# skywoodsz/qm_control

Measured on NVIDIA H100. Metric: mpc_wbc_iters_per_s, higher is better.
Workload: dtype f64

## Files before the change

### qm_control_b200/csrc/kernels/mpc_kernels.cu

```cuda
#include <cstdlib>
#include "mpc_api.cuh"
#include "mpc_device.cuh"
#include "node_eval.cuh"
#include "wlinalg.cuh"

namespace qmb {

#ifndef QMB_LQ_WARPS
#define QMB_LQ_WARPS 4
#endif
#ifndef QMB_LQ_MINB
#define QMB_LQ_MINB 4
#endif
constexpr int LQ_WARPS = QMB_LQ_WARPS, LS_WARPS = 4, SETUP_WARPS = 4;
enum { MST_ITER_CAP = 1, MST_OVERFLOW = 2, MST_NAN = 4, MST_NOT_PD = 8, MST_NO_STEP = 16, MST_CONVERGED = 32, MST_NEG_DT = 64 };

__device__ __forceinline__ double interval_start(double t, int ev) { return ev == 2 ? t + WEAK_EPS : t; }
__device__ __forceinline__ double interval_end(double t, int ev) { return ev == 1 ? t - WEAK_EPS : t; }
__device__ __forceinline__ int clamp_events(int ne) { return ne < 0 ? 0 : (ne > EMAX ? EMAX : ne); }
__device__ __forceinline__ int clamp_targets(int nk) { return nk < 1 ? 1 : (nk > KMAX ? KMAX : nk); }
__device__ __forceinline__ int flag_mask(int mode) { int m = 0; for (int i = 0; i < 4; ++i) if (contact_flag(mode, i)) m |= 1 << i; return m; }

struct SetupIdx { int iu, ix; double au, ax; };
__host__ __device__ inline size_t setup_smem_per_warp(int nmax) { return (size_t)nmax * (8 + 8 + 4 + sizeof(SetupIdx) + 4) + 8 * EMAX + 64; }
// ... 259 lines not shown
  const double dyn_ss = warp_sum(bb * bb);
  if (lane < NX) {
    const int c = lane; double a1[9], out[9];
#pragma unroll
    for (int q = 0; q < 9; ++q) a1[q] = sm.A1r[q * NX + c];
#pragma unroll
    for (int r = 0; r < 9; ++r) { const double* a2 = sm.Ar + r * NX; double aa = 0.0;
#pragma unroll
      for (int q = 0; q < 9; ++q) aa = fma(a2[3 + q], a1[q], aa);
      out[r] = dt * (w1 * a1[r] + w2 * (a2[c] + cdt * aa));
      if (c < 12) { double b1 = 0.0, b2 = 0.0; if (r < 3) { b1 = b1v[r < 3 ? r : 0]; b2 = b2v[r < 3 ? r : 0]; } double ab = a2[c % 3] * imass;
#pragma unroll
        for (int q = 0; q < 3; ++q) ab += a2[3 + q] * b1v[q]; lt.BrdF[r * 12 + c] = dt * (w1 * b1 + w2 * (b2 + cdt * ab)); }
      else if (r < 3) lt.BrdJ[r * NJ + c - 12] = dt * w2 * cdt * a2[c]; }
#pragma unroll
    for (int r = 0; r < 9; ++r) sm.A1r[r * NX + c] = out[r];
  }
  __syncwarp();
  double* tl = sg + ST_TAIL; int32_t* si = reinterpret_cast<int32_t*>(tl + T_INT);
  if (lane < NX) {
    const int r = lane; double bt = lt.bvec[r];
    if (r >= 3 && r < 6) {
      double* arow = sm.A1r + (r - 3) * NX; double acc[12];
#pragma unroll
      for (int i = 0; i < 4; ++i) { const LegWs& L = sm.leg[i];
#pragma unroll
        for (int c = 0; c < 12; ++c) acc[c] = 0.0;
        for (int j = 0; j < 3; ++j) if (L.dep[j]) { const double coef = lt.BrdJ[(r - 3) * NJ + L.first + j]; bt += coef * L.Pe[j];
#pragma unroll
          for (int c = 0; c < 12; ++c) acc[c] = fma(coef, L.Px[j][c], acc[c]); }
#pragma unroll
        for (int c = 0; c < 12; ++c) arow[sup_col(c, L.first)] += acc[c];
      }
    }
    if (r >= 12 && r < 24) {
      const int i = foot_of_leg_joint(lfp, r - 12); const LegWs& L = sm.leg[i]; const int j = (r - 12) % 3;
      if (L.dep[j]) bt += dtw * L.Pe[j];
    }
    if (r < 3) for (int f = 0; f < 4; ++f) bt += (dtw * imass) * sm.Pe_full[3 * f + r];
    if (r >= 3 && r < 12) for (int f = 0; f < 4; ++f) if (!sm.leg[f].stance) for (int a = 0; a < 3; ++a) bt += lt.BrdF[(r - 3) * 12 + 3 * f + a] * sm.Pe_full[3 * f + a];
    tl[T_b + r] = bt;
    if (r >= 3 && r < 12) sg[ST_AR + (r - 3) * LDX + NX] = bt;
  }
  if (lane >= 3 && lane < 12) sm.A1r[(lane - 3) * NX + lane] += 1.0;
  __syncwarp();
#pragma unroll
  for (int r = 0; r < 9; ++r) { if (lane < NX) sg[ST_AR + r * LDX + lane] = sm.A1r[r * NX + lane]; else if (lane == 31) sg[ST_AR + r * LDX + 31] = 0.0; }
  for (int e = lane; e < 36; e += 32) sg[ST_AR + (e >> 2) * LDX + 32 + (e & 3)] = 0.0;
  for (int e = lane; e < 144; e += 32) { const int j12 = e / 12, c = e - 12 * j12; const LegWs& L = sm.leg[foot_of_leg_joint(lfp, j12)]; const int j = j12 % 3; tl[T_PXJ + e] = L.dep[j] ? L.Px[j][c] : 0.0; }
  for (int e = lane; e < 9 * LDB; e += 32) {
    const int rr = e / LDB, a = e - rr * LDB; const int r = 3 + rr; double v = 0.0;
    if (a < m) { const int fa = sm.free_idx[a];
      if (fa < 12) v = lt.BrdF[rr * 12 + fa];
      else if (r < 6) { v = lt.BrdJ[rr * NJ + fa - 12];
        if (fa < 24) { const LegWs& L = sm.leg[foot_of_leg_joint(lfp, fa - 12)]; if (!L.stance) { const int jf = (fa - 12) % 3; v += lt.BrdJ[rr * NJ + L.first + L.pivot] * L.Pu2[jf > L.pivot ? jf - 1 : jf]; } } }
    }
    sg[ST_BR + e] = v;
  }
  if (lane < NX) {
    const int r = lane; double acc[NX];
    if (mdl->q_is_diag) { const double qrr = mdl->Qdiag[r];
#pragma unroll
      for (int c = 0; c < NX; ++c) acc[c] = (c == r) ? qrr : 0.0; }
    else {
#pragma unroll
      for (int c = 0; c < NX; ++c) acc[c] = mdl->Q[r * NX + c]; }
    double qv = sm.quad.qf[r];
    const int ea = ee_pos(r);
    if (ea >= 0) {
#pragma unroll
      for (int c = 0; c < 6; ++c) { acc[6 + c] += sm.quad.E[ea * 12 + c]; acc[24 + c] += sm.quad.E[ea * 12 + 6 + c]; }
    }
#pragma unroll
    for (int i = 0; i < 4; ++i) {
      const LegWs& L = sm.leg[i]; const int first = L.first;
      const int pr = (r < 6) ? r : ((r >= 9 && r < 12) ? r - 3 : ((r >= 12 + first && r < 15 + first) ? 9 + r - 12 - first : -1));
      if (pr >= 0) {
        double blk[12];
#pragma unroll
        for (int c = 0; c < 12; ++c) blk[c] = 0.0;
        double w3[3] = {0.0, 0.0, 0.0};
        for (int j = 0; j < 3; ++j) if (L.dep[j]) { const double pj = L.Px[j][pr]; qv = fma(pj, L.rs[j], qv);
#pragma unroll
          for (int a = 0; a < 3; ++a) w3[a] = fma(pj, L.Rl[3 * j + a], w3[a]); }
        for (int a = 0; a < 3; ++a) if (L.dep[a]) { const double wa = w3[a];
#pragma unroll
          for (int c = 0; c < 12; ++c) blk[c] = fma(wa, L.Px[a][c], blk[c]); }
#pragma unroll
        for (int c = 0; c < 6; ++c) acc[c] += blk[c];
#pragma unroll
        for (int c = 0; c < 3; ++c) acc[9 + c] += blk[6 + c];
#pragma unroll
        for (int l = 0; l < 4; ++l) if (first == 3 * l) {
#pragma unroll
          for (int c = 0; c < 3; ++c) acc[12 + 3 * l + c] += blk[9 + c]; }
      }
    }
    const double dq = sm.quad.qdiag[r];
#pragma unroll
    for (int c = 0; c < NX; ++c) if (r <= c) sg[ST_Q + q_row_offset(c) + r] = dt * (acc[c] + ((c == r) ? dq : 0.0));
    if (!(r & 1)) sg[ST_Q + q_row_offset(r) + r + 1] = 0.0;
    tl[T_q + r] = dt * qv;
  }
  for (int e = lane; e < 8 * 12; e += 32) tl[T_SJ + e] = 0.0;
  __syncwarp();
  if (lane < MU) {
    const int a = lane; double rt[3] = {0.0, 0.0, 0.0}; double rtil = 0.0;
    if (a < m) {
      const int fa = sm.free_idx[a]; double rv = sm.rs[fa]; int li = -1, jf = -1;
      if (fa >= 12 && fa < 24) { li = foot_of_leg_joint(lfp, fa - 12); jf = (fa - 12) % 3; }
      const bool swing_joint = li >= 0 && !sm.leg[li].stance;
      if (swing_joint) {
        const LegWs& L = sm.leg[li]; const int pv = L.pivot; const int jfi = jf > pv ? jf - 1 : jf; const double pu = L.Pu2[jfi];
        rv += pu * L.rs[pv];
        const double coef = L.Rl[3 * jf + pv]; double* Srow = tl + T_SJ + (2 * li + jfi) * 12;
        const double cf = dt * (coef + pu * L.Rl[3 * pv + pv]);
        for (int c = 0; c < 12; ++c) Srow[c] = cf * L.Px[pv][c];
      }
      rtil = dt * rv;
      if (fa >= 24) rt[0] = dt * quad_R(mdl, &sm.quad, fa, fa);
      else { const int bi = fa / 3;
        for (int jc = 0; jc < 3; ++jc) { const int fc = 3 * bi + jc; if (sm.col_of_input[fc] < 0) continue;
          double v = quad_R(mdl, &sm.quad, fa, fc);
          if (swing_joint) { const LegWs& L = sm.leg[li]; const int pv = L.pivot; const double pa = L.Pu2[jf > pv ? jf - 1 : jf], pc = L.Pu2[jc > pv ? jc - 1 : jc];
            v += pa * L.Rl[3 * pv + jc] + L.Rl[3 * jf + pv] * pc + pa * L.Rl[3 * pv + pv] * pc; }
          rt[jc] = dt * v; } }
    }
    tl[T_r + a] = rtil; tl[T_RT + 3 * a] = rt[0]; tl[T_RT + 3 * a + 1] = rt[1]; tl[T_RT + 3 * a + 2] = rt[2];
  }
  if (lane < 4) { const LegWs& L = sm.leg[lane]; tl[T_PU2 + 2 * lane] = L.Pu2[0]; tl[T_PU2 + 2 * lane + 1] = L.Pu2[1]; si[SI_PIV + lane] = L.stance ? -1 : L.pivot;
    int nf = 0; for (int jj = 0; jj < 3; ++jj) if (!L.stance && jj != L.pivot) si[SI_PCOL + 2 * lane + nf++] = L.free_col[jj]; if (L.stance) { si[SI_PCOL + 2 * lane] = -1; si[SI_PCOL + 2 * lane + 1] = -1; } }
  if (lane < MAXDEP) { const int d = lane; double pe = 0.0; int di = -1; if (d < ndep) { di = sm.dep_idx[d]; pe = sm.Pe_full[di]; } tl[T_PED + d] = pe; si[SI_DEP + d] = di; }
  if (lane < MU) si[SI_FREE + lane] = (lane < m) ? sm.free_idx[lane] : -1;
  if (lane == 0) { si[SI_TYPE] = 0; si[SI_M] = m; si[SI_NDEP] = ndep; tl[T_MISC] = dtw; tl[T_MISC + 1] = dt * cost_val; tl[T_MISC + 2] = dt * dyn_ss; tl[T_MISC + 3] = dt * eq_ss; }
}

#ifndef QMB_TMA
#define QMB_TMA 1
#endif
constexpr int RIC_THREADS = 128, RIC_NTYPE = 512;
struct RicSmem {
  double P[NX * LDX];
  double A[NX * LDX];
  double W[NX * LDX];
  double Bm[NX * LDB], PB[NX * LDB];
  double G[MU * LDG];
  double H[MU * LDH];
  double Lt[MU * MU];
  alignas(16) double tail[TAIL_DBL];
  double dx[32], dut[32], tmp[32];
  double red[RIC_THREADS / 32][4];
  alignas(8) unsigned long long bar[4];
  int flag; int pad_;
  signed char srow[MU + 2], sfirst[MU + 2];
  unsigned char ntype[RIC_NTYPE];
};
static_assert(sizeof(RicSmem) <= 57344 - 64, "Riccati kernel must keep four CTAs per SM");

__device__ __forceinline__ unsigned smem_u32(const void* p) { return (unsigned)__cvta_generic_to_shared(p); }
__device__ __forceinline__ void mbar_init(unsigned long long* b, unsigned count) { asm volatile("mbarrier.init.shared::cta.b64 [%0], %1;\n" ::"r"(smem_u32(b)), "r"(count) : "memory"); }
__device__ __forceinline__ void mbar_expect_tx(unsigned long long* b, unsigned bytes) { asm volatile("mbarrier.arrive.expect_tx.shared::cta.b64 _, [%0], %1;\n" ::"r"(smem_u32(b)), "r"(bytes) : "memory"); }
__device__ __forceinline__ void mbar_wait(unsigned long long* b, unsigned parity) {
  asm volatile("{\n .reg .pred p;\n WAIT_LOOP:\n mbarrier.try_wait.parity.shared::cta.b64 p, [%0], %1;\n @p bra WAIT_DONE;\n bra WAIT_LOOP;\n WAIT_DONE:\n}\n" ::"r"(smem_u32(b)), "r"(parity) : "memory");
}
__device__ __forceinline__ void bulk_g2s(void* dst, const void* src, unsigned bytes, unsigned long long* bar) {
  asm volatile("cp.async.bulk.shared::cluster.global.mbarrier::complete_tx::bytes [%0], [%1], %2, [%3];\n" ::"r"(smem_u32(dst)), "l"(src), "r"(bytes), "r"(smem_u32(bar)) : "memory");
}
__device__ __forceinline__ void cp_async16(void* smem_dst, const void* gmem_src) { asm volatile("cp.async.cg.shared.global [%0], [%1], 16;\n" ::"r"(smem_u32(smem_dst)), "l"(gmem_src) : "memory"); }
__device__ __forceinline__ void cp_async_wait_all() { asm volatile("cp.async.wait_all;\n" ::: "memory"); }
struct CopyGroup {
  unsigned long long* bar; unsigned phase;
  __device__ __forceinline__ void begin(unsigned bytes, int tid) { if (QMB_TMA && tid == 0) mbar_expect_tx(bar, bytes); }
  __device__ __forceinline__ void copy(void* dst, const void* src, unsigned bytes, int tid, int nthr = RIC_THREADS, int t0 = 0) {
    if (QMB_TMA) { if (tid == 0) bulk_g2s(dst, src, bytes, bar); }
    else { const int me = tid - t0; if (me >= 0 && me < nthr) for (unsigned o = 16u * me; o < bytes; o += 16u * nthr) cp_async16((char*)dst + o, (const char*)src + o); }
  }
  __device__ __forceinline__ void wait() { if (QMB_TMA) mbar_wait(bar, phase & 1u); else { cp_async_wait_all(); __syncthreads(); } ++phase; }
  __device__ __forceinline__ void skip() { ++phase; }
};

__device__ __forceinline__ void dmma884(double (&c)[2], double a, double b) {
  asm("mma.sync.aligned.m8n8k4.row.col.f64.f64.f64.f64 {%0,%1}, {%2}, {%3}, {%0,%1};\n" : "+d"(c[0]), "+d"(c[1]) : "d"(a), "d"(b));
}
template <int K, int MT, int NT, bool NEG>
__device__ __forceinline__ void warp_mma(const double* __restrict__ X, int ldx, int i0, const double* __restrict__ Y, int ldy, int j0, double (&c)[MT][NT][2], int g, int t) {
#pragma unroll
  for (int ks = 0; ks < (K + 3) / 4; ++ks) {
    const int kr = 4 * ks + t; const bool ok = (4 * ks + 3 < K) || (kr < K);
    double a[MT], bf[NT];
#pragma unroll
    for (int m = 0; m < MT; ++m) { const double v = ok ? X[kr * ldx + i0 + 8 * m + g] : 0.0; a[m] = NEG ? -v : v; }
#pragma unroll
    for (int n = 0; n < NT; ++n) bf[n] = ok ? Y[kr * ldy + j0 + 8 * n + g] : 0.0;
#pragma unroll
    for (int m = 0; m < MT; ++m)
#pragma unroll
      for (int n = 0; n < NT; ++n) dmma884(c[m][n], a[m], bf[n]);
  }
}
template <int MT, int NT>
__device__ __forceinline__ void cfrag_load(const double* M, int ld, int i0, int j0, int rows, double (&c)[MT][NT][2], int g, int t) {
#pragma unroll
  for (int m = 0; m < MT; ++m)
#pragma unroll
    for (int n = 0; n < NT; ++n) { const int ri = i0 + 8 * m + g;
      if (ri < rows) { const double2 v = *reinterpret_cast<const double2*>(M + ri * ld + j0 + 8 * n + 2 * t); c[m][n][0] = v.x; c[m][n][1] = v.y; } else { c[m][n][0] = 0.0; c[m][n][1] = 0.0; } }
}
template <int MT, int NT>
__device__ __forceinline__ void cfrag_store(double* M, int ld, int i0, int j0, int rows, const double (&c)[MT][NT][2], int g, int t) {
#pragma unroll
  for (int m = 0; m < MT; ++m)
#pragma unroll
    for (int n = 0; n < NT; ++n) { const int ri = i0 + 8 * m + g; if (ri < rows) *reinterpret_cast<double2*>(M + ri * ld + j0 + 8 * n + 2 * t) = make_double2(c[m][n][0], c[m][n][1]); }
}
__device__ __forceinline__ int sup_pos(int j, int first) { return j < 6 ? j : ((j >= 9 && j < 12) ? j - 3 : (((unsigned)(j - 12 - first) < 3u) ? 9 + j - 12 - first : -1)); }

__global__ void __launch_bounds__(RIC_THREADS, 4) mpc_riccati_kernel(const DevModel* __restrict__ mdl, int b0, int B, int nmax, MpcProblemDev p, MpcSolutionDev sol, const double* __restrict__ stage,
                                                                  double* __restrict__ gains, double* __restrict__ dxo, double* __restrict__ duo, double* __restrict__ robot, int32_t* __restrict__ status) {
  extern __shared__ __align__(16) unsigned char smem_raw[];
  RicSmem& sm = *reinterpret_cast<RicSmem*>(smem_raw);
  const int tid = threadIdx.x, warp = tid >> 5, lane = tid & 31, ti = tid >> 2, jb = tid & 3; const int b = b0 + blockIdx.x;
  if (status[b] & MST_CONVERGED) return;
  const int n = sol.n_nodes[b]; const int N = n - 1;
  const double* sgb = stage + (size_t)b * nmax * STAGE_DBL; double* gb = gains + (size_t)b * nmax * GAIN_DBL;
  const int lfp = pack_leg_foot(mdl); const double imass = 1.0 / mdl->total_mass;
  for (int e = tid; e < (int)(sizeof(RicSmem) / 8); e += RIC_THREADS) reinterpret_cast<double*>(&sm)[e] = 0.0;
  __syncthreads();
  if (tid < NX && (tid < 3 || tid >= 24)) sm.A[tid * LDX + tid] = 1.0;
  if (tid == 0) { for (int i = 0; i < 4; ++i) mbar_init(&sm.bar[i], 1); asm volatile("fence.mbarrier_init.release.cluster;\n" ::: "memory"); }
  asm volatile("fence.proxy.async.shared::cta;\n" ::: "memory");
  const bool types_in_smem = n <= RIC_NTYPE;
  auto rec_type = [&](int k) -> int { return reinterpret_cast<const int32_t*>(sgb + (size_t)k * STAGE_DBL + ST_TAIL + T_INT)[SI_TYPE]; };
  if (types_in_smem) for (int k = tid; k < n; k += RIC_THREADS) sm.ntype[k] = (unsigned char)rec_type(k);
  auto node_type = [&](int k) -> int { return types_in_smem ? (int)sm.ntype[k] : rec_type(k); };
  CopyGroup gAB{&sm.bar[0], 0u}, gT{&sm.bar[1], 0u}, gQ{&sm.bar[2], 0u}, gF1{&sm.bar[3], 0u};
  auto issue_ab = [&](int k) { const double* sg = sgb + (size_t)k * STAGE_DBL; gAB.begin((9 * LDX + 9 * LDB) * 8, tid);
    gAB.copy(sm.A + 3 * LDX, sg + ST_AR, 9 * LDX * 8, tid); gAB.copy(sm.Bm + 3 * LDB, sg + ST_BR, 9 * LDB * 8, tid); };
  auto issue_tail = [&](int k) { gT.begin(TAIL_DBL * 8, tid); gT.copy(sm.tail, sgb + (size_t)k * STAGE_DBL + ST_TAIL, TAIL_DBL * 8, tid); };
  auto issue_q = [&](int k) { gQ.begin(Q_PACKED * 8, tid); gQ.copy(sm.Bm, sgb + (size_t)k * STAGE_DBL + ST_Q, Q_PACKED * 8, tid); };
  auto expand = [&]() {
    const double* tl = sm.tail; const int32_t* si = reinterpret_cast<const int32_t*>(tl + T_INT); const double dtw = tl[T_MISC];
    for (int e = tid; e < 144; e += RIC_THREADS) { const int j12 = e / 12, c = e - 12 * j12; const int col = sup_col(c, 3 * (j12 / 3));
      sm.A[(12 + j12) * LDX + col] = ((col == 12 + j12) ? 1.0 : 0.0) + dtw * tl[T_PXJ + e]; }
    if (tid < NX && (tid < 3 || tid >= 12)) sm.A[tid * LDX + NX] = tl[T_b + tid];
    for (int e = tid; e < 21 * MU; e += RIC_THREADS) {
      const int rr = e / MU, a = e - rr * MU; const int r = rr < 3 ? rr : rr + 9; const int fa = si[SI_FREE + a]; double v = 0.0;
      if (fa >= 0) {
        if (r < 3) { if (fa < 12 && fa - 3 * (fa / 3) == r) v = dtw * imass; }
        else if (fa == r) v = dtw;
        else if (fa >= 12 && fa < 24) { const int j = fa - 12, lg = j / 3, foot = (lfp >> (2 * lg)) & 3; const int pv = si[SI_PIV + foot];
          if (pv >= 0 && r == 12 + 3 * lg + pv) { const int jf = j - 3 * lg; v = dtw * tl[T_PU2 + 2 * foot + (jf > pv ? jf - 1 : jf)]; } }
      }
      sm.Bm[r * LDB + a] = v;
    }
    if (tid < MU) { const int fa = si[SI_FREE + tid]; int slot = -1, first = 0;
      if (fa >= 12 && fa < 24) { const int j = fa - 12, lg = j / 3, foot = (lfp >> (2 * lg)) & 3; const int pv = si[SI_PIV + foot]; if (pv >= 0) { const int jf = j - 3 * lg; slot = 2 * foot + (jf > pv ? jf - 1 : jf); first = 3 * lg; } }
      sm.srow[tid] = (signed char)slot; sm.sfirst[tid] = (signed char)first; }
  };
  for (int e = tid; e < NX * NX; e += RIC_THREADS) { const int r = e / NX, c = e - r * NX; sm.P[r * LDX + c] = sgb[(size_t)N * STAGE_DBL + ST_Q + q_row_offset(r > c ? r : c) + (r > c ? c : r)]; }
  if (tid < NX) sm.P[tid * LDX + NX] = sgb[(size_t)N * STAGE_DBL + ST_TAIL + T_q + tid];
  double perf0 = 0, perf1 = 0, perf2 = 0;
  for (int k = tid; k < n; k += RIC_THREADS) { const double* pf = sgb + (size_t)k * STAGE_DBL + ST_TAIL + T_MISC + 1; perf0 += pf[0]; perf1 += pf[1]; perf2 += pf[2]; }
  if (tid < NX) { const double d = p.x0[(size_t)b * NX + tid] - sol.x[(size_t)b * nmax * NX + tid]; sm.dx[tid] = d; perf1 += d * d; }
  perf0 = warp_sum(perf0); perf1 = warp_sum(perf1); perf2 = warp_sum(perf2);
  if (lane == 0) { sm.red[warp][0] = perf0; sm.red[warp][1] = perf1; sm.red[warp][2] = perf2; }
  __syncthreads();
  double perf[3]; for (int i = 0; i < 3; ++i) perf[i] = sm.red[0][i] + sm.red[1][i] + sm.red[2][i] + sm.red[3][i];
  if (N >= 1) { issue_tail(N - 1); if (node_type(N - 1) != 1) issue_ab(N - 1); gT.wait(); if (node_type(N - 1) != 1) expand(); }
  int st = 0;
  const int g = lane >> 2, t = lane & 3;
  for (int k = N - 1; k >= 0; --k) {
    const int type = node_type(k); const int tnext = k > 0 ? node_type(k - 1) : 1;
    if (type == 1) {
      __syncthreads();
      if (tid < NX) { double sv = sm.P[tid * LDX + NX]; for (int j = 0; j < NX; ++j) sv = fma(sm.P[tid * LDX + j], sm.tail[T_b + j], sv); sm.tmp[tid] = sv; }
      __syncthreads();
      if (tid < NX) sm.P[tid * LDX + NX] = sm.tmp[tid];
      if (k > 0) { issue_tail(k - 1); if (tnext != 1) issue_ab(k - 1); gT.wait(); if (tnext != 1) expand(); }
      continue;
    }
    gAB.wait(); if (QMB_TMA) __syncthreads();
    const double dtw_k = sm.tail[T_MISC]; const int acol0 = reinterpret_cast<const int32_t*>(sm.tail + T_INT)[SI_M] - 6;
    { const int i0 = 16 * (warp >> 1), j0 = 16 * (warp & 1);
      double c[2][2][2] = {};
      if (warp & 1) {
#pragma unroll
        for (int m = 0; m < 2; ++m) { const int ri = i0 + 8 * m + g; if (ri < NX) {
            if (t < 3) { c[m][1][0] = sm.P[(24 + 2 * t) * LDX + ri]; c[m][1][1] = sm.P[(25 + 2 * t) * LDX + ri]; }
            else { double sv = sm.P[ri * LDX + NX];
#pragma unroll
              for (int kk = 24; kk < NX; ++kk) sv = fma(sm.P[kk * LDX + ri], sm.A[kk * LDX + NX], sv);
              c[m][1][0] = sv; } } } }
      warp_mma<24, 2, 2, false>(sm.P, LDX, i0, sm.A, LDX, j0, c, g, t);
      cfrag_store<2, 2>(sm.W, LDX, i0, j0, NX, c, g, t);
      double d[1][3][2];
#pragma unroll
      for (int nn = 0; nn < 3; ++nn)
#pragma unroll
        for (int e = 0; e < 2; ++e) { const int a = 8 * nn + 2 * t + e - acol0, ri = 8 * warp + g; d[0][nn][e] = ((unsigned)a < 6u && ri < NX) ? dtw_k * sm.P[(24 + a) * LDX + ri] : 0.0; }
      warp_mma<24, 1, 3, false>(sm.P, LDX, 8 * warp, sm.Bm, LDB, 0, d, g, t);
      cfrag_store<1, 3>(sm.PB, LDB, 8 * warp, 0, NX, d, g, t); }
    __syncthreads();
    if (tid < NX) sm.P[tid * LDX + NX] = sm.tail[T_q + tid];
    { const double* tl = sm.tail; const int32_t* si = reinterpret_cast<const int32_t*>(tl + T_INT); const int mm = si[SI_M];
      double c[3][1][2];
#pragma unroll
      for (int mt = 0; mt < 3; ++mt) { const int a = 8 * mt + g; const bool rowok = a < MU; const int slot = rowok ? sm.srow[a] : -1, first = rowok ? sm.sfirst[a] : 0;
#pragma unroll
        for (int e = 0; e < 2; ++e) { const int j = 8 * warp + 2 * t + e; double v = 0.0;
          if (rowok) { if (j == NX) v = tl[T_r + a]; else if (slot >= 0 && j < NX) { const int ps = sup_pos(j, first); if (ps >= 0) v = tl[T_SJ + slot * 12 + ps]; }
            if ((unsigned)(a - acol0) < 6u) v = fma(dtw_k, sm.W[(24 + a - acol0) * LDX + j], v); }
          c[mt][0][e] = v; } }
      warp_mma<24, 3, 1, false>(sm.Bm, LDB, 0, sm.W, LDX, 8 * warp, c, g, t); cfrag_store<3, 1>(sm.G, LDG, 0, 8 * warp, MU, c, g, t);
      if (warp < 3) { double d[3][1][2];
#pragma unroll
        for (int mt = 0; mt < 3; ++mt) { const int a = 8 * mt + g; const int fa = (a < MU) ? si[SI_FREE + a] : -1;
#pragma unroll
          for (int e = 0; e < 2; ++e) { const int cc = 8 * warp + 2 * t + e; double v = 0.0;
            if (a < MU && cc < MU) { if (a >= mm) v = (a == cc) ? 1.0 : 0.0;
              else if (fa >= 24) v = (a == cc) ? tl[T_RT + 3 * a] : 0.0;
              else { const int fc = si[SI_FREE + cc]; if (fc >= 0 && fc / 3 == fa / 3) v = tl[T_RT + 3 * a + fc - 3 * (fc / 3)]; }
              if ((unsigned)(a - acol0) < 6u) v = fma(dtw_k, sm.PB[(24 + a - acol0) * LDB + cc], v); }
            d[mt][0][e] = v; } }
        warp_mma<24, 3, 1, false>(sm.Bm, LDB, 0, sm.PB, LDB, 8 * warp, d, g, t); cfrag_store<3, 1>(sm.H, LDH, 0, 8 * warp, MU, d, g, t); } }
    __syncthreads();
    issue_q(k);
    if (k > 0) issue_tail(k - 1);
    const int sw = (k + b) & 3;
    if (!QMB_TMA) gQ.wait();
    if (warp == sw) {
      if (QMB_TMA) gQ.skip();
      double hr[MU], y[MU]; double dinv = 0.0; bool ok = true; double* Yb = sm.PB;
#pragma unroll
      for (int c = 0; c < MU; ++c) { hr[c] = (lane < MU) ? sm.H[c * LDH + lane] : 0.0; y[c] = sm.G[c * LDG + lane]; }
#pragma unroll
      for (int j = 0; j < MU; ++j) {
        const double djj = __shfl_sync(FULL, hr[j], j); if (!(djj > 0.0)) ok = false;
        const double inv = rsqrt(djj); const double lij = hr[j] * inv;
        if (lane == j) dinv = inv;
        if (lane < MU) sm.Lt[j * MU + lane] = lij;
        y[j] *= inv; Yb[j * LDX + lane] = y[j];
#pragma unroll
        for (int c = j + 1; c < MU; ++c) { const double lcj = __shfl_sync(FULL, lij, c); hr[c] = fma(-lij, lcj, hr[c]); y[c] = fma(-lcj, y[j], y[c]); }
      }
      if (lane < MU) sm.dut[lane] = dinv;
      if (!ok && lane == 0) sm.flag = 1;
      __syncwarp();
      double* gk = gb + (size_t)k * GAIN_DBL;
#pragma unroll
      for (int a = MU - 1; a >= 0; --a) {
        asm volatile("" ::: "memory");
        y[a] *= sm.dut[a];
        gk[a * LDG + lane] = -y[a];
#pragma unroll
        for (int c = 0; c < a; ++c) y[c] = fma(-sm.Lt[c * MU + a], y[a], y[c]);
      }
    } else {
      if (QMB_TMA) gQ.wait();
      const int hi = (warp - sw - 1) & 3;
      for (int tile = hi; tile < 16; tile += 3) { const int i0 = 8 * (tile >> 2), j0 = 8 * (tile & 3);
        double c[1][1][2]; const int ri = i0 + g;
#pragma unroll
        for (int e = 0; e < 2; ++e) { const int cj = j0 + 2 * t + e; double v = (ri < NX && cj <= NX) ? (cj == NX ? sm.P[ri * LDX + NX] : (cj <= ri ? sm.Bm[q_row_offset(ri) + cj] : sm.Bm[q_row_offset(cj) + ri])) : 0.0;
          if (ri >= 24 && ri < NX && cj <= NX) v += sm.W[ri * LDX + cj];
          c[0][0][e] = v; }
        warp_mma<24, 1, 1, false>(sm.A, LDX, i0, sm.W, LDX, j0, c, g, t); cfrag_store<1, 1>(sm.P, LDX, i0, j0, NX, c, g, t); }
    }
    __syncthreads();
    if (sm.flag) { st |= MST_NOT_PD; if (k > 0) gT.wait(); break; }
    if (k > 0) { if (tnext != 1) issue_ab(k - 1); gT.wait(); if (tnext != 1) expand(); }
    { const double* Yb = sm.PB; const int i0 = 16 * (warp >> 1), j0 = 16 * (warp & 1);
      double c[2][2][2]; cfrag_load<2, 2>(sm.P, LDX, i0, j0, NX, c, g, t); warp_mma<MU, 2, 2, true>(Yb, LDX, i0, Yb, LDX, j0, c, g, t); cfrag_store<2, 2>(sm.P, LDX, i0, j0, NX, c, g, t); }
  }
  __syncthreads();
  double armijo = 0.0, dxn2 = 0.0, dun2 = 0.0;
  if (!(st & MST_NOT_PD)) {
    auto issue_fwd = [&](int k) {
      if (k >= N) return; const int o = k & 1; CopyGroup& cg = o ? gF1 : gAB; const double* sg = sgb + (size_t)k * STAGE_DBL; const bool ev = node_type(k) == 1;
      cg.begin((ev ? 0 : (GAIN_DBL + 9 * LDX + 9 * LDB) * 8) + TAIL_DBL * 8, tid);
      cg.copy((o ? sm.P : sm.A) + 9 * LDX, sg + ST_TAIL, TAIL_DBL * 8, tid);
      if (!ev) { cg.copy(o ? sm.W : sm.G, gb + (size_t)k * GAIN_DBL, GAIN_DBL * 8, tid); cg.copy(o ? sm.P : sm.A, sg + ST_AR, 9 * LDX * 8, tid); cg.copy(o ? sm.PB : sm.Bm, sg + ST_BR, 9 * LDB * 8, tid); } };
    issue_fwd(0);
    for (int k = 0; k < N; ++k) {
      const int o = k & 1; const double* Kb = o ? sm.W : sm.G; const double* ARb = o ? sm.P : sm.A; const double* BRb = o ? sm.PB : sm.Bm; const double* tl = (o ? sm.P : sm.A) + 9 * LDX;
      double* dxk = dxo + ((size_t)b * nmax + k) * NX; double* duk = duo + ((size_t)b * nmax + k) * NU;
      const double* dxc = (k & 1) ? sm.tmp : sm.dx; double* dxn = (k & 1) ? sm.dx : sm.tmp;
      if (o) gF1.wait(); else gAB.wait();
      if (QMB_TMA) __syncthreads();
      issue_fwd(k + 1);
      const int32_t* si = reinterpret_cast<const int32_t*>(tl + T_INT); const int type = si[SI_TYPE], ndep = si[SI_NDEP], mm = si[SI_M]; const double dtw = tl[T_MISC];
      if (tid < NX) { const double dxi = dxc[tid]; dxk[tid] = dxi; dxn2 += dxi * dxi; }
      if (type == 1) { if (tid < NX) { duk[tid] = 0.0; dxn[tid] = dxc[tid] + tl[T_b + tid]; } continue; }
      { double s = 0.0;
        if (ti < MU) { const double* kr = Kb + ti * LDG + jb * 8; const double* dx = dxc + jb * 8;
#pragma unroll
          for (int v = 0; v < 8; ++v) s = fma(kr[v], dx[v], s); }
        s += __shfl_xor_sync(FULL, s, 1); s += __shfl_xor_sync(FULL, s, 2); if (ti < MU && jb == 0) sm.dut[ti] = s + Kb[ti * LDG + NX]; }
      __syncthreads();
      {
        static_assert(MAXDEP * 8 == RIC_THREADS, "one 8-thread group per dependent input");
        const int d = tid >> 3, q8 = tid & 7; double s = 0.0; const int di = (d < ndep) ? si[SI_DEP + d] : -1;
        if (di >= 12) { const int j = di - 12, lg = j / 3, first = 3 * lg; const double* px = tl + T_PXJ + j * 12;
          s = px[q8] * dxc[sup_col(q8, first)]; if (q8 < 4) s = fma(px[q8 + 8], dxc[sup_col(q8 + 8, first)], s);
          if (q8 >= 4 && q8 < 6) { const int foot = (lfp >> (2 * lg)) & 3; const int col = si[SI_PCOL + 2 * foot + q8 - 4]; if (si[SI_PIV + foot] >= 0 && col >= 0) s = fma(tl[T_PU2 + 2 * foot + q8 - 4], sm.dut[col], s); } }
        s += __shfl_xor_sync(FULL, s, 1); s += __shfl_xor_sync(FULL, s, 2); s += __shfl_xor_sync(FULL, s, 4);
        if (di >= 0 && q8 == 0) { const double full = s + tl[T_PED + d]; duk[di] = full; dun2 += full * full; if (di >= 12) dxn[di] = dxc[di] + dtw * s + tl[T_b + di]; } }
      if (tid < NX) armijo += tl[T_q + tid] * dxc[tid];
      if (tid < MU) { const double dut = sm.dut[tid]; armijo += tl[T_r + tid] * dut; const int fi = si[SI_FREE + tid];
        if (fi >= 0) { duk[fi] = dut; dun2 += dut * dut; if (fi >= 12) dxn[fi] = dxc[fi] + dtw * dut + tl[T_b + fi]; } }
      if (warp == 1 && lane < 3) { double acc = 0.0; for (int a = 0; a < mm; ++a) { const int fa = si[SI_FREE + a]; if (fa < 12 && fa - 3 * (fa / 3) == lane) acc += sm.dut[a]; }
        dxn[lane] = dxc[lane] + dtw * imass * acc + tl[T_b + lane]; }
      if (warp >= 2) { const int rr = (tid - 64) >> 2; double s = 0.0;
        if (rr < 9) { const double* ar = ARb + rr * LDX + jb * 8; const double* dx = dxc + jb * 8;
#pragma unroll
          for (int v = 0; v < 8; ++v) s = fma(ar[v], dx[v], s);
          if (jb < 3) { const double* br = BRb + rr * LDB + jb * 8; const double* du = sm.dut + jb * 8;
#pragma unroll
            for (int v = 0; v < 8; ++v) s = fma(br[v], du[v], s); } }
        s += __shfl_xor_sync(FULL, s, 1); s += __shfl_xor_sync(FULL, s, 2); if (rr < 9 && jb == 0) dxn[3 + rr] = s + tl[T_b + 3 + rr]; }
    }
    __syncthreads();
    if (tid < NX) { const double dxi = ((N & 1) ? sm.tmp : sm.dx)[tid]; dxo[((size_t)b * nmax + N) * NX + tid] = dxi; duo[((size_t)b * nmax + N) * NU + tid] = 0.0; dxn2 += dxi * dxi; armijo += sgb[(size_t)N * STAGE_DBL + ST_TAIL + T_q + tid] * dxi; }
  }
  armijo = warp_sum(armijo); dxn2 = warp_sum(dxn2); dun2 = warp_sum(dun2);
  __syncthreads();
  if (lane == 0) { sm.red[warp][0] = armijo; sm.red[warp][1] = dxn2; sm.red[warp][2] = dun2; }
  __syncthreads();
  if (tid == 0) { double a = 0, x2 = 0, u2 = 0; for (int w = 0; w < RIC_THREADS / 32; ++w) { a += sm.red[w][0]; x2 += sm.red[w][1]; u2 += sm.red[w][2]; }
    double* rb = robot + (size_t)b * ROBOT_DBL; rb[0] = a; rb[1] = perf[0]; rb[2] = perf[1]; rb[3] = perf[2]; rb[4] = sqrt(x2); rb[5] = sqrt(u2); if (st) atomicOr(&status[b], st); }
}

__device__ __forceinline__ void fixup_inputs(MpcSolutionDev sol, int b, int nmax, int n, int tid, int nthreads) {
  const int32_t* ge = sol.event + (size_t)b * nmax; double* gu = sol.u + (size_t)b * nmax * NU;
  for (int i = tid; i < NU; i += nthreads) for (int k = 1; k < n; ++k) if ((k == n - 1) || (ge[k] == 1)) gu[(size_t)k * NU + i] = gu[(size_t)(k - 1) * NU + i];
}

#ifndef QMB_LS_MINB
#define QMB_LS_MINB 4
#endif
__global__ void __launch_bounds__(32 * LS_WARPS, QMB_LS_MINB) mpc_linesearch_kernel(const DevModel* __restrict__ mdl, int b0, int B, int nmax, MpcProblemDev p, MpcSolutionDev sol, const double* __restrict__ dxo, const double* __restrict__ duo,
                                                                     const double* __restrict__ robot, int32_t* __restrict__ status, double* __restrict__ step_info, int iteration) {
  __shared__ double red[LS_WARPS][3]; __shared__ int decision; __shared__ double s_ev[EMAX]; __shared__ unsigned char s_modes[EMAX + 8];
  const int tid = threadIdx.x, warp = tid >> 5, lane = tid & 31; const int b = b0 + blockIdx.x; if (b >= B) return;
  if (status[b] & MST_CONVERGED) return;
  const int n = sol.n_nodes[b]; const int N = n - 1;
  const double* gt = sol.t + (size_t)b * nmax; const int32_t* ge = sol.event + (size_t)b * nmax;
  double* gx = sol.x + (size_t)b * nmax * NX; double* gu = sol.u + (size_t)b * nmax * NU; const double* gdx = dxo + (size_t)b * nmax * NX; const double* gdu = duo + (size_t)b * nmax * NU;
  const int ne = clamp_events(p.n_events[b]); const double* ev = s_ev; const unsigned char* modes = s_modes;
  if (tid < 32) { const double* gev = p.event_times + (size_t)b * EMAX; const int32_t* gmodes = p.modes + (size_t)b * (EMAX + 1); s_ev[lane] = (lane < ne) ? gev[lane] : 0.0; s_modes[lane] = (unsigned char)((lane <= ne) ? gmodes[lane] : 15); if (lane == 0) s_modes[EMAX] = (unsigned char)((EMAX <= ne) ? gmodes[EMAX] : 15); }
  __syncthreads();
  const int nk = clamp_targets(p.n_target[b]); const double* tt = p.target_times + (size_t)b * KMAX; const double* ts = p.target_states + (size_t)b * KMAX * TARGET_DIM;
  const double* rb = robot + (size_t)b * ROBOT_DBL; const double armijo = rb[0], base_cost = rb[1], base_viol = sqrt(rb[2] + rb[3]), dxn = rb[4], dun = rb[5];
  const bool failed = (status[b] & MST_NOT_PD) != 0;
  double alpha = 1.0; bool accepted = false; double sc = base_cost, sd = rb[2], se = rb[3];
  const double w1 = mdl->rk_w1, w2 = mdl->rk_w2;
  while (!failed) {
    double cost = 0.0, dyn = 0.0, eq = 0.0;
    for (int k = tid; k <= N; k += 32 * LS_WARPS) {
      double xa[NX], ua[NU]; const bool terminal = (k == N);
#pragma unroll
      for (int i = 0; i < NX; ++i) { xa[i] = gx[(size_t)k * NX + i] + alpha * gdx[(size_t)k * NX + i]; ua[i] = terminal ? 0.0 : gu[(size_t)k * NU + i] + alpha * gdu[(size_t)k * NU + i]; }
      if (k == 0) { double s = 0.0; for (int i = 0; i < NX; ++i) { const double d = p.x0[(size_t)b * NX + i] - xa[i]; s = fma(d, d, s); } dyn += s; }
      if (!terminal && ge[k] == 1) { double s = 0.0; for (int i = 0; i < NX; ++i) { const double d = xa[i] - (gx[(size_t)(k + 1) * NX + i] + alpha * gdx[(size_t)(k + 1) * NX + i]); s = fma(d, d, s); } dyn += s; continue; }
      const double t = interval_start(gt[k], ge[k]);
      const double dt = terminal ? 1.0 : interval_end(gt[k + 1], ge[k + 1]) - t; const int mode = mode_at_time(ev, modes, ne, t); const int fm = terminal ? 0 : flag_mask(mode);
      ne::BaseKin bk; ne::FlowAcc acc; double f1[12];
      ne::base_eval<false>(mdl, xa, bk); ne::flow_acc_init(acc);
      { double fe[4][3], pf[4][3];
#pragma unroll 1
        for (int i = 0; i < 4; ++i) { double d[3], Jl[9]; ne::foot_eval<false>(mdl, xa, ua, bk, i, acc, d, pf[i], Jl, nullptr, nullptr); if (!terminal) ne::foot_velocity_1<false>(mdl, xa, ua, bk, i, d, Jl, nullptr, fe[i], nullptr); }
        if (!terminal) eq += dt * ne::equality_ss(mdl, ua, fe, pf, fm, ev, modes, ne, t, nullptr); }
      ne::flow_finish<false>(mdl, xa, bk, acc, f1, nullptr);
      { const ne::TargetSeg sg = ne::target_segment(tt, ts, nk, t); double pref[3], qref[4], ee[6]; ne::target_pose(sg, nk, pref, qref); ne::ee_eval<false>(mdl, xa, bk, pref, qref, ee, nullptr);
        cost += dt * ne::cost_value(mdl, xa, ua, sg, ee, fm, terminal); }
      if (terminal) continue;
      const double cdt = mdl->rk_c * dt;
#pragma unroll
      for (int i = 0; i < NX; ++i) xa[i] += cdt * (i < 12 ? f1[i < 12 ? i : 0] : ua[i]);
      double f2[12]; ne::base_eval<false>(mdl, xa, bk); ne::flow_acc_init(acc);
#pragma unroll 1
      for (int i = 0; i < 4; ++i) { double d[3]; ne::foot_eval<false>(mdl, xa, ua, bk, i, acc, d, nullptr, nullptr, nullptr, nullptr); }
      ne::flow_finish<false>(mdl, xa, bk, acc, f2, nullptr);
      double s = 0.0;
#pragma unroll
      for (int i = 0; i < NX; ++i) { const double fa = (i < 12) ? f1[i < 12 ? i : 0] : ua[i], fb = (i < 12) ? f2[i < 12 ? i : 0] : ua[i];
        const double x0i = gx[(size_t)k * NX + i] + alpha * gdx[(size_t)k * NX + i];
        const double d = x0i + dt * (w1 * fa + w2 * fb) - (gx[(size_t)(k + 1) * NX + i] + alpha * gdx[(size_t)(k + 1) * NX + i]); s = fma(d, d, s); }
      dyn += dt * s;
    }
    cost = warp_sum(cost); dyn = warp_sum(dyn); eq = warp_sum(eq);
    if (lane == 0) { red[warp][0] = cost; red[warp][1] = dyn; red[warp][2] = eq; }
    __syncthreads();
    if (threadIdx.x == 0) {
      double c = 0, dd = 0, e = 0; for (int w = 0; w < LS_WARPS; ++w) { c += red[w][0]; dd += red[w][1]; e += red[w][2]; }
      const double sv = sqrt(dd + e), am = alpha * armijo; bool acc;
      if (sv > mdl->g_max) acc = sv < (1.0 - mdl->gamma_c) * base_viol;
      else if (sv < mdl->g_min && base_viol < mdl->g_min && am < 0.0) acc = c < base_cost + mdl->armijo_factor * am;
      else acc = (c < base_cost - mdl->gamma_c * base_viol) || (sv < (1.0 - mdl->gamma_c) * base_viol);
      red[0][0] = c; red[0][1] = dd; red[0][2] = e;
      int dec = 0; if (acc) dec = 1; else { const double an = alpha * mdl->alpha_decay; if ((an * dxn < mdl->delta_tol && an * dun < mdl->delta_tol) || an < mdl->alpha_min) dec = 2; }
      decision = dec;
    }
    __syncthreads();
    const int dec = decision; sc = red[0][0]; sd = red[0][1]; se = red[0][2];
    __syncthreads();
    if (dec == 1) { accepted = true; break; }
    if (dec == 2) break;
    alpha *= mdl->alpha_decay;
  }
  if (accepted) {
    const int tot = n * NX, totu = N * NU, nt = blockDim.x;
    for (int e0 = threadIdx.x; e0 < tot; e0 += 4 * nt) {
      double vx[4], vu[4];
#pragma unroll
      for (int q = 0; q < 4; ++q) { const int e = e0 + q * nt; vx[q] = (e < tot) ? gx[e] + alpha * gdx[e] : 0.0; vu[q] = (e < totu) ? gu[e] + alpha * gdu[e] : 0.0; }
#pragma unroll
      for (int q = 0; q < 4; ++q) { const int e = e0 + q * nt; if (e < tot) gx[e] = vx[q]; if (e < totu) gu[e] = vu[q]; }
    }
  } else { alpha = 0.0; sc = base_cost; sd = rb[2]; se = rb[3]; }
  __syncthreads();
  fixup_inputs(sol, b, nmax, n, threadIdx.x, blockDim.x);
  if (threadIdx.x == 0) {
    int flags = accepted ? 0 : MST_NO_STEP;
    if (iteration + 1 < mdl->sqp_iterations) {
      const bool stepsize = alpha < mdl->alpha_min;
      const bool metrics = fabs(sc - base_cost) < mdl->cost_tol && sqrt(sd + se) < mdl->g_min;
// ... 242 lines not shown
```

Baseline: 19.29.

## Overlap Riccati back-solve with next-stage prefetch and G/H decode via named barriers

Restructures the backward Riccati loop so the Cholesky warp writes gains after the block barrier, while the other three warps issue the next stage's A/B copy, expand it, and pre-decode the G/H constraint matrices into shared memory, coordinated through named barriers. The P -= Y^T Y update is split into 8x8 tiles across the three non-Cholesky warps, and the gain triangular solve runs alongside it on the Cholesky warp. This is meant to take the serial per-stage setup and gain back-substitution off the critical path. It adds named-barrier and async-proxy synchronization complexity, including extra TMA waits and a proxy fence, which risks ordering bugs or warp imbalance.

```diff
diff --git a/qm_control_b200/csrc/kernels/mpc_kernels.cu b/qm_control_b200/csrc/kernels/mpc_kernels.cu
--- a/qm_control_b200/csrc/kernels/mpc_kernels.cu
+++ b/qm_control_b200/csrc/kernels/mpc_kernels.cu
@@ -435,7 +435,6 @@
   double red[RIC_THREADS / 32][4];
   alignas(8) unsigned long long bar[4];
   int flag; int pad_;
-  signed char srow[MU + 2], sfirst[MU + 2];
   unsigned char ntype[RIC_NTYPE];
 };
 static_assert(sizeof(RicSmem) <= 57344 - 64, "Riccati kernel must keep four CTAs per SM");
@@ -451,6 +450,8 @@
 }
 __device__ __forceinline__ void cp_async16(void* smem_dst, const void* gmem_src) { asm volatile("cp.async.cg.shared.global [%0], [%1], 16;\n" ::"r"(smem_u32(smem_dst)), "l"(gmem_src) : "memory"); }
 __device__ __forceinline__ void cp_async_wait_all() { asm volatile("cp.async.wait_all;\n" ::: "memory"); }
+__device__ __forceinline__ void named_bar_sync(int id, int n) { asm volatile("bar.sync %0, %1;\n" ::"r"(id), "r"(n) : "memory"); }
+__device__ __forceinline__ void named_bar_arrive(int id, int n) { asm volatile("bar.arrive %0, %1;\n" ::"r"(id), "r"(n) : "memory"); }
 struct CopyGroup {
   unsigned long long* bar; unsigned phase;
   __device__ __forceinline__ void begin(unsigned bytes, int tid) { if (QMB_TMA && tid == 0) mbar_expect_tx(bar, bytes); }
@@ -517,16 +518,16 @@
   if (types_in_smem) for (int k = tid; k < n; k += RIC_THREADS) sm.ntype[k] = (unsigned char)rec_type(k);
   auto node_type = [&](int k) -> int { return types_in_smem ? (int)sm.ntype[k] : rec_type(k); };
   CopyGroup gAB{&sm.bar[0], 0u}, gT{&sm.bar[1], 0u}, gQ{&sm.bar[2], 0u}, gF1{&sm.bar[3], 0u};
-  auto issue_ab = [&](int k) { const double* sg = sgb + (size_t)k * STAGE_DBL; gAB.begin((9 * LDX + 9 * LDB) * 8, tid);
-    gAB.copy(sm.A + 3 * LDX, sg + ST_AR, 9 * LDX * 8, tid); gAB.copy(sm.Bm + 3 * LDB, sg + ST_BR, 9 * LDB * 8, tid); };
+  auto issue_ab = [&](int k, int me, int nthr) { const double* sg = sgb + (size_t)k * STAGE_DBL; gAB.begin((9 * LDX + 9 * LDB) * 8, me);
+    gAB.copy(sm.A + 3 * LDX, sg + ST_AR, 9 * LDX * 8, me, nthr); gAB.copy(sm.Bm + 3 * LDB, sg + ST_BR, 9 * LDB * 8, me, nthr); };
   auto issue_tail = [&](int k) { gT.begin(TAIL_DBL * 8, tid); gT.copy(sm.tail, sgb + (size_t)k * STAGE_DBL + ST_TAIL, TAIL_DBL * 8, tid); };
   auto issue_q = [&](int k) { gQ.begin(Q_PACKED * 8, tid); gQ.copy(sm.Bm, sgb + (size_t)k * STAGE_DBL + ST_Q, Q_PACKED * 8, tid); };
-  auto expand = [&]() {
+  auto expand = [&](int me, int nthr) {
     const double* tl = sm.tail; const int32_t* si = reinterpret_cast<const int32_t*>(tl + T_INT); const double dtw = tl[T_MISC];
-    for (int e = tid; e < 144; e += RIC_THREADS) { const int j12 = e / 12, c = e - 12 * j12; const int col = sup_col(c, 3 * (j12 / 3));
+    for (int e = me; e < 144; e += nthr) { const int j12 = e / 12, c = e - 12 * j12; const int col = sup_col(c, 3 * (j12 / 3));
       sm.A[(12 + j12) * LDX + col] = ((col == 12 + j12) ? 1.0 : 0.0) + dtw * tl[T_PXJ + e]; }
-    if (tid < NX && (tid < 3 || tid >= 12)) sm.A[tid * LDX + NX] = tl[T_b + tid];
-    for (int e = tid; e < 21 * MU; e += RIC_THREADS) {
+    if (me < NX && (me < 3 || me >= 12)) sm.A[me * LDX + NX] = tl[T_b + me];
+    for (int e = me; e < 21 * MU; e += nthr) {
       const int rr = e / MU, a = e - rr * MU; const int r = rr < 3 ? rr : rr + 9; const int fa = si[SI_FREE + a]; double v = 0.0;
       if (fa >= 0) {
         if (r < 3) { if (fa < 12 && fa - 3 * (fa / 3) == r) v = dtw * imass; }
@@ -536,9 +537,29 @@
       }
       sm.Bm[r * LDB + a] = v;
     }
-    if (tid < MU) { const int fa = si[SI_FREE + tid]; int slot = -1, first = 0;
-      if (fa >= 12 && fa < 24) { const int j = fa - 12, lg = j / 3, foot = (lfp >> (2 * lg)) & 3; const int pv = si[SI_PIV + foot]; if (pv >= 0) { const int jf = j - 3 * lg; slot = 2 * foot + (jf > pv ? jf - 1 : jf); first = 3 * lg; } }
-      sm.srow[tid] = (signed char)slot; sm.sfirst[tid] = (signed char)first; }
+  };
+  auto decode = [&](int me, int nthr, int it0, int it1) {
+    const double* tl = sm.tail; const int32_t* si = reinterpret_cast<const int32_t*>(tl + T_INT); const int mm = si[SI_M];
+    for (int it = it0 + me; it < it1; it += nthr) {
+      if (it < 4 * MU) {
+        const int a = it >> 2, j0 = 8 * (it & 3); const int fa = si[SI_FREE + a]; int slot = -1, first = 0;
+        if (fa >= 12 && fa < 24) { const int j = fa - 12, lg = j / 3, foot = (lfp >> (2 * lg)) & 3; const int pv = si[SI_PIV + foot]; if (pv >= 0) { const int jf = j - 3 * lg; slot = 2 * foot + (jf > pv ? jf - 1 : jf); first = 3 * lg; } }
+        double* gr = sm.G + a * LDG + j0;
+#pragma unroll
+        for (int jj = 0; jj < 8; ++jj) { const int j = j0 + jj; double v = 0.0;
+          if (j == NX) v = tl[T_r + a]; else if (slot >= 0 && j < NX) { const int ps = sup_pos(j, first); if (ps >= 0) v = tl[T_SJ + slot * 12 + ps]; }
+          gr[jj] = v; }
+      } else {
+        const int a = (it - 4 * MU) / 3, c0 = 8 * ((it - 4 * MU) % 3); const int fa = si[SI_FREE + a];
+        double* hr = sm.H + a * LDH + c0;
+#pragma unroll
+        for (int jj = 0; jj < 8; ++jj) { const int cc = c0 + jj; double v = 0.0;
+          if (cc < MU) { if (a >= mm) v = (a == cc) ? 1.0 : 0.0;
+            else if (fa >= 24) v = (a == cc) ? tl[T_RT + 3 * a] : 0.0;
+            else { const int fc = si[SI_FREE + cc]; if (fc >= 0 && fc / 3 == fa / 3) v = tl[T_RT + 3 * a + fc - 3 * (fc / 3)]; } }
+          hr[jj] = v; }
+      }
+    }
   };
   for (int e = tid; e < NX * NX; e += RIC_THREADS) { const int r = e / NX, c = e - r * NX; sm.P[r * LDX + c] = sgb[(size_t)N * STAGE_DBL + ST_Q + q_row_offset(r > c ? r : c) + (r > c ? c : r)]; }
   if (tid < NX) sm.P[tid * LDX + NX] = sgb[(size_t)N * STAGE_DBL + ST_TAIL + T_q + tid];
@@ -549,7 +570,7 @@
   if (lane == 0) { sm.red[warp][0] = perf0; sm.red[warp][1] = perf1; sm.red[warp][2] = perf2; }
   __syncthreads();
   double perf[3]; for (int i = 0; i < 3; ++i) perf[i] = sm.red[0][i] + sm.red[1][i] + sm.red[2][i] + sm.red[3][i];
-  if (N >= 1) { issue_tail(N - 1); if (node_type(N - 1) != 1) issue_ab(N - 1); gT.wait(); if (node_type(N - 1) != 1) expand(); }
+  if (N >= 1) { issue_tail(N - 1); if (node_type(N - 1) != 1) issue_ab(N - 1, tid, RIC_THREADS); gT.wait(); if (node_type(N - 1) != 1) { expand(tid, RIC_THREADS); decode(tid, RIC_THREADS, 0, 7 * MU); } }
   int st = 0;
   const int g = lane >> 2, t = lane & 3;
   for (int k = N - 1; k >= 0; --k) {
@@ -559,7 +580,7 @@
       if (tid < NX) { double sv = sm.P[tid * LDX + NX]; for (int j = 0; j < NX; ++j) sv = fma(sm.P[tid * LDX + j], sm.tail[T_b + j], sv); sm.tmp[tid] = sv; }
       __syncthreads();
       if (tid < NX) sm.P[tid * LDX + NX] = sm.tmp[tid];
-      if (k > 0) { issue_tail(k - 1); if (tnext != 1) issue_ab(k - 1); gT.wait(); if (tnext != 1) expand(); }
+      if (k > 0) { issue_tail(k - 1); if (tnext != 1) issue_ab(k - 1, tid, RIC_THREADS); gT.wait(); if (tnext != 1) { expand(tid, RIC_THREADS); decode(tid, RIC_THREADS, 0, 7 * MU); } }
       continue;
     }
     gAB.wait(); if (QMB_TMA) __syncthreads();
@@ -585,37 +606,33 @@
       cfrag_store<1, 3>(sm.PB, LDB, 8 * warp, 0, NX, d, g, t); }
     __syncthreads();
     if (tid < NX) sm.P[tid * LDX + NX] = sm.tail[T_q + tid];
-    { const double* tl = sm.tail; const int32_t* si = reinterpret_cast<const int32_t*>(tl + T_INT); const int mm = si[SI_M];
-      double c[3][1][2];
-#pragma unroll
-      for (int mt = 0; mt < 3; ++mt) { const int a = 8 * mt + g; const bool rowok = a < MU; const int slot = rowok ? sm.srow[a] : -1, first = rowok ? sm.sfirst[a] : 0;
-#pragma unroll
-        for (int e = 0; e < 2; ++e) { const int j = 8 * warp + 2 * t + e; double v = 0.0;
-          if (rowok) { if (j == NX) v = tl[T_r + a]; else if (slot >= 0 && j < NX) { const int ps = sup_pos(j, first); if (ps >= 0) v = tl[T_SJ + slot * 12 + ps]; }
-            if ((unsigned)(a - acol0) < 6u) v = fma(dtw_k, sm.W[(24 + a - acol0) * LDX + j], v); }
-          c[mt][0][e] = v; } }
+    { double c[3][1][2]; cfrag_load<3, 1>(sm.G, LDG, 0, 8 * warp, MU, c, g, t);
+#pragma unroll
+      for (int mt = 0; mt < 3; ++mt) { const int a = 8 * mt + g;
+        if (a < MU && (unsigned)(a - acol0) < 6u) {
+#pragma unroll
+          for (int e = 0; e < 2; ++e) c[mt][0][e] = fma(dtw_k, sm.W[(24 + a - acol0) * LDX + 8 * warp + 2 * t + e], c[mt][0][e]); } }
       warp_mma<24, 3, 1, false>(sm.Bm, LDB, 0, sm.W, LDX, 8 * warp, c, g, t); cfrag_store<3, 1>(sm.G, LDG, 0, 8 * warp, MU, c, g, t);
-      if (warp < 3) { double d[3][1][2];
-#pragma unroll
-        for (int mt = 0; mt < 3; ++mt) { const int a = 8 * mt + g; const int fa = (a < MU) ? si[SI_FREE + a] : -1;
-#pragma unroll
-          for (int e = 0; e < 2; ++e) { const int cc = 8 * warp + 2 * t + e; double v = 0.0;
-            if (a < MU && cc < MU) { if (a >= mm) v = (a == cc) ? 1.0 : 0.0;
-              else if (fa >= 24) v = (a == cc) ? tl[T_RT + 3 * a] : 0.0;
-              else { const int fc = si[SI_FREE + cc]; if (fc >= 0 && fc / 3 == fa / 3) v = tl[T_RT + 3 * a + fc - 3 * (fc / 3)]; }
-              if ((unsigned)(a - acol0) < 6u) v = fma(dtw_k, sm.PB[(24 + a - acol0) * LDB + cc], v); }
-            d[mt][0][e] = v; } }
+      if (warp < 3) { double d[3][1][2]; cfrag_load<3, 1>(sm.H, LDH, 0, 8 * warp, MU, d, g, t);
+#pragma unroll
+        for (int mt = 0; mt < 3; ++mt) { const int a = 8 * mt + g;
+          if (a < MU && (unsigned)(a - acol0) < 6u) {
+#pragma unroll
+            for (int e = 0; e < 2; ++e) { const int cc = 8 * warp + 2 * t + e; if (cc < MU) d[mt][0][e] = fma(dtw_k, sm.PB[(24 + a - acol0) * LDB + cc], d[mt][0][e]); } } }
         warp_mma<24, 3, 1, false>(sm.Bm, LDB, 0, sm.PB, LDB, 8 * warp, d, g, t); cfrag_store<3, 1>(sm.H, LDH, 0, 8 * warp, MU, d, g, t); } }
     __syncthreads();
     issue_q(k);
     if (k > 0) issue_tail(k - 1);
     const int sw = (k + b) & 3;
+    const bool fetch = k > 0 && tnext != 1;
     if (!QMB_TMA) gQ.wait();
+    double y[MU];
     if (warp == sw) {
       if (QMB_TMA) gQ.skip();
-      double hr[MU], y[MU]; double dinv = 0.0; bool ok = true; double* Yb = sm.PB;
+      double hr[MU]; double dinv = 0.0; bool ok = true; double* Yb = sm.PB;
 #pragma unroll
       for (int c = 0; c < MU; ++c) { hr[c] = (lane < MU) ? sm.H[c * LDH + lane] : 0.0; y[c] = sm.G[c * LDG + lane]; }
+      if (fetch) named_bar_arrive(2, RIC_THREADS);
 #pragma unroll
       for (int j = 0; j < MU; ++j) {
         const double djj = __shfl_sync(FULL, hr[j], j); if (!(djj > 0.0)) ok = false;
@@ -628,16 +645,6 @@
       }
       if (lane < MU) sm.dut[lane] = dinv;
       if (!ok && lane == 0) sm.flag = 1;
-      __syncwarp();
-      double* gk = gb + (size_t)k * GAIN_DBL;
-#pragma unroll
-      for (int a = MU - 1; a >= 0; --a) {
-        asm volatile("" ::: "memory");
-        y[a] *= sm.dut[a];
-        gk[a * LDG + lane] = -y[a];
-#pragma unroll
-        for (int c = 0; c < a; ++c) y[c] = fma(-sm.Lt[c * MU + a], y[a], y[c]);
-      }
     } else {
       if (QMB_TMA) gQ.wait();
       const int hi = (warp - sw - 1) & 3;
@@ -648,13 +655,36 @@
           if (ri >= 24 && ri < NX && cj <= NX) v += sm.W[ri * LDX + cj];
           c[0][0][e] = v; }
         warp_mma<24, 1, 1, false>(sm.A, LDX, i0, sm.W, LDX, j0, c, g, t); cfrag_store<1, 1>(sm.P, LDX, i0, j0, NX, c, g, t); }
+      if (k > 0) { if (QMB_TMA) gT.wait(); else gT.skip(); }
+      if (fetch) {
+        const int me = 32 * hi + lane;
+        named_bar_sync(1, 96);
+        issue_ab(k - 1, me, 96); expand(me, 96);
+        named_bar_sync(2, RIC_THREADS);
+        decode(me, 96, 0, 7 * MU);
+      }
     }
     __syncthreads();
-    if (sm.flag) { st |= MST_NOT_PD; if (k > 0) gT.wait(); break; }
-    if (k > 0) { if (tnext != 1) issue_ab(k - 1); gT.wait(); if (tnext != 1) expand(); }
-    { const double* Yb = sm.PB; const int i0 = 16 * (warp >> 1), j0 = 16 * (warp & 1);
-      double c[2][2][2]; cfrag_load<2, 2>(sm.P, LDX, i0, j0, NX, c, g, t); warp_mma<MU, 2, 2, true>(Yb, LDX, i0, Yb, LDX, j0, c, g, t); cfrag_store<2, 2>(sm.P, LDX, i0, j0, NX, c, g, t); }
-  }
+    const bool npd = sm.flag != 0;
+    if (warp == sw) {
+      double* gk = gb + (size_t)k * GAIN_DBL;
+#pragma unroll
+      for (int a = MU - 1; a >= 0; --a) {
+        asm volatile("" ::: "memory");
+        y[a] *= sm.dut[a];
+        gk[a * LDG + lane] = -y[a];
+#pragma unroll
+        for (int c = 0; c < a; ++c) y[c] = fma(-sm.Lt[c * MU + a], y[a], y[c]);
+      }
+      if (k > 0) { if (QMB_TMA) gT.wait(); else gT.skip(); }
+    } else if (!npd) {
+      const int hi = (warp - sw - 1) & 3; const double* Yb = sm.PB;
+      for (int tile = hi; tile < 16; tile += 3) { const int i0 = 8 * (tile >> 2), j0 = 8 * (tile & 3);
+        double c[1][1][2]; cfrag_load<1, 1>(sm.P, LDX, i0, j0, NX, c, g, t); warp_mma<MU, 1, 1, true>(Yb, LDX, i0, Yb, LDX, j0, c, g, t); cfrag_store<1, 1>(sm.P, LDX, i0, j0, NX, c, g, t); }
+    }
+    if (npd) { st |= MST_NOT_PD; if (fetch) gAB.wait(); break; }
+  }
+  asm volatile("fence.proxy.async;\n" ::: "memory");
   __syncthreads();
   double armijo = 0.0, dxn2 = 0.0, dun2 = 0.0;
   if (!(st & MST_NOT_PD)) {
```

Measured after the change: 19.68 (median of 6 runs). 2.0% higher.
